# VisualComputingInstitute/RovinaSemanticSegmentation

Hardware: AMD Instinct MI355X
Metric: Mpix/s RF+5-iter DenseCRF @640x480 RGB-D (higher is better)
Workload: dtype f32; 1 GPU; BASELINE configs[2]: batch of 64 synthetic 640x480 RGB-D key frames per GPU (10 % invalid-depth holes: yes; 2 input sets in rotation), 4-tree forest (2^14 leaves/tree, D=366, C=9), RF + 5-iter DenseCRF (d=6, Potts w=10), marginals + labels written to HBM; label_gather=none

## Files before the change

### rovinasemanticsegmentation_amd/csrc/kernels_lattice.hip

```cpp
#include <string.h>

#include <rocprim/rocprim.hpp>

#include "device_math.h"
#include "rvseg_crf.h"

namespace rvseg {

constexpr int ST_EMPTY = -1, ST_LOCKED = -2, ST_FILLED = 0;

struct Key8 {
    union {
        short k[8];
        unsigned w[4];
        unsigned long long q[2];
    };
};

__device__ __forceinline__ unsigned hash_key(const Key8& key) {
    unsigned h = 0x9E3779B9u;
#pragma unroll
    for (int i = 0; i < 4; i++) {
        h ^= key.w[i];
        h *= 0x85EBCA6Bu;
// ... 249 lines not shown
    }
    RV_LAUNCHED("lattice_points_kernel");
}

struct SlotFilled {
    __device__ __forceinline__ int operator()(int st) const { return st == ST_FILLED ? 1 : 0; }
};

__global__ void __launch_bounds__(256)
lattice_compact_kernel(LatticeDev L) {
    const unsigned slot = blockIdx.x * blockDim.x + threadIdx.x;
    if (slot >= L.cap_total) return;
    const bool filled = L.state[slot] == ST_FILLED;
    const int id = L.slot_to_id[slot];
    if (filled && (unsigned)id < (unsigned)L.m_bound) {
        L.vkeys[2 * (size_t)id] = L.tkeys[2 * (size_t)slot];
        L.vkeys[2 * (size_t)id + 1] = L.tkeys[2 * (size_t)slot + 1];
    }
    const unsigned cap_f = L.cap_f_mask + 1;
    if ((slot & L.cap_f_mask) == 0) L.fstart[slot >> L.cap_f_log2] = id;
    if (slot == L.cap_total - 1) {
        const int M = id + (filled ? 1 : 0);
        L.counters[0] = M;
        L.fstart[L.n_frames] = M;
        if (M > L.m_bound) L.counters[1] = 1;
    }
    if ((slot & L.cap_f_mask) == L.cap_f_mask) {
        const int first = L.slot_to_id[slot - L.cap_f_mask];
        const int Mf = id + (filled ? 1 : 0) - first;
        if ((unsigned)Mf > cap_f / 2) L.counters[1] = 1;
    }
}

__global__ void __launch_bounds__(256)
lattice_remap_kernel(LatticeDev L, unsigned* __restrict__ sort_keys, unsigned* __restrict__ sort_vals, long long n_entries) {
    const long long e = (long long)blockIdx.x * blockDim.x + threadIdx.x;
    if (e >= n_entries) return;
    int id = L.slot_to_id[L.offsets[e]];
    id = id < L.m_bound ? id : L.m_bound - 1;
    L.offsets[e] = id;
    sort_keys[e] = (unsigned)id;
    sort_vals[e] = (unsigned)e;
}

__global__ void __launch_bounds__(256)
lattice_neighbours_kernel(LatticeDev L) {
    const long long gid = (long long)blockIdx.x * blockDim.x + threadIdx.x;
    const int M = L.counters[0] < L.m_bound ? L.counters[0] : L.m_bound;
    const int d = L.d;
    if (gid >= (long long)M * (d + 1)) return;
    const int j = (int)(gid / M);
    const int id = (int)(gid - (long long)j * M);
    Key8 key;
    const unsigned long long* src = L.vkeys + 2 * (size_t)id;
    key.q[0] = src[0];
    key.q[1] = src[1];
    Key8 n1 = key, n2 = key;
    for (int k = 0; k < d; k++) { n1.k[k] = (short)(key.k[k] - 1); n2.k[k] = (short)(key.k[k] + 1); }
    if (j < d) { n1.k[j] = (short)(key.k[j] + d); n2.k[j] = (short)(key.k[j] - d); }
    const unsigned fbase = (unsigned)(unsigned short)key.k[7] << L.cap_f_log2;
    const int s1 = hash_lookup(L.state, L.tkeys, fbase, L.cap_f_mask, n1);
    const int s2 = hash_lookup(L.state, L.tkeys, fbase, L.cap_f_mask, n2);
    L.nb1[(size_t)j * L.m_bound + id] = s1 < 0 ? -1 : L.slot_to_id[s1];
    L.nb2[(size_t)j * L.m_bound + id] = s2 < 0 ? -1 : L.slot_to_id[s2];
}

__global__ void __launch_bounds__(256)
lattice_csr_kernel(LatticeDev L, const unsigned* __restrict__ keys_sorted, const unsigned* __restrict__ vals_sorted,
                   long long n_entries) {
    const long long k = (long long)blockIdx.x * blockDim.x + threadIdx.x;
    if (k >= n_entries) return;
    const unsigned e = vals_sorted[k];
    const unsigned key = keys_sorted[k];
    L.csr_pw[k] = make_uint2(e / (unsigned)(L.d + 1), __float_as_uint(L.bary[e]));
    if (k == 0 || keys_sorted[k - 1] != key) L.vstart[key] = (unsigned)k;
    if (k == n_entries - 1 || keys_sorted[k + 1] != key) L.vend[key] = (unsigned)(k + 1);
}

void launch_vertex_order(const LatticeDev& L, SortBuffers& sb, hipStream_t s);

constexpr int CS_PIX_MIN = 256;
constexpr int CS_MCAP = 4096;

template <bool SCATTER>
__global__ void __launch_bounds__(256)
csr_pass_kernel(LatticeDev L, unsigned* __restrict__ bh, int wbpf, int mcap) {
    extern __shared__ unsigned cs_cnt[];
    const int wave = threadIdx.x >> 6, lane = threadIdx.x & 63;
    const long long gwb = (long long)blockIdx.x * 4 + wave;
    const int frame = (int)(gwb / wbpf);
    if (frame >= L.n_frames) return;
    const int wb = (int)(gwb - (long long)frame * wbpf);
    const int f0 = L.fstart[frame] < L.m_bound ? L.fstart[frame] : L.m_bound;
    const int f1 = L.fstart[frame + 1] < L.m_bound ? L.fstart[frame + 1] : L.m_bound;
    const int Mf = f1 - f0 < mcap ? f1 - f0 : mcap;
    const unsigned n_entries_total = (unsigned)((long long)L.n_frames * L.N * (L.d + 1));
    unsigned* my = cs_cnt + (size_t)wave * mcap;
    unsigned* row = bh + (size_t)wbpf * f0 + (size_t)wb * Mf;
    for (int lv = lane; lv < Mf; lv += 64) my[lv] = SCATTER ? row[lv] : 0u;
    if (Mf == 0 && lane == 0) my[0] = 0xFFFFFFFFu;
    __builtin_amdgcn_fence(__ATOMIC_SEQ_CST, "wavefront");
    const int dp1 = L.d + 1;
    const long long p0 = (long long)wb * L.cs_pix;
    const long long p1 = p0 + L.cs_pix < L.N ? p0 + L.cs_pix : L.N;
    const long long ebeg = ((long long)frame * L.N + p0) * dp1, eend = ((long long)frame * L.N + p1) * dp1;
    const unsigned long long lt = lane == 0 ? 0ull : (~0ull >> (64 - lane));
    auto fetch = [&](long long e, int& id, float& wgt) {
        id = 0; wgt = 0.f;
        if (e < eend) {
            if (!SCATTER) { id = L.slot_to_id[L.offsets[e]]; id = id < L.m_bound ? id : L.m_bound - 1; }
            else { id = L.offsets[e]; wgt = L.bary[e]; }
        }
    };
    int id_n; float w_n;
    fetch(ebeg + lane, id_n, w_n);
    for (long long base = ebeg; base < eend; base += 64) {
        const long long e = base + lane;
        const bool valid = e < eend;
        const int id = id_n;
        const float wgt = w_n;
        fetch(e + 64, id_n, w_n);
        if (!SCATTER && valid) L.offsets[e] = id;
        int lv = valid ? id - f0 : -1;
        if (lv >= Mf) lv = Mf - 1;
        if (valid && lv < 0) lv = 0;
        if (!SCATTER) {
            if (valid) atomicAdd(&my[lv], 1u);
            continue;
        }
        bool pending = valid;
        for (;;) {
            const unsigned long long todo = __ballot(pending);
            if (!todo) break;
            const int leader = __ffsll((long long)todo) - 1;
            const int k = __shfl(lv, leader, 64);
            const bool same = pending && lv == k;
            const unsigned long long m = __ballot(same);
            const unsigned c = (unsigned)__popcll(m);
            if (SCATTER) {
                const unsigned b = my[k];
                if (same) {
                    const unsigned pos = b + (unsigned)__popcll(m & lt);
                    if (pos < n_entries_total) {
                        L.csr_pw[pos] = make_uint2((unsigned)(e / dp1), __float_as_uint(wgt));
                    }
                }
                if (lane == leader) my[k] = b + c;
            } else {
                if (lane == leader) my[k] = my[k] + c;
            }
            pending = pending && !same;
        }
        __builtin_amdgcn_fence(__ATOMIC_SEQ_CST, "wavefront");
    }
    if (!SCATTER) {
        for (int lv = lane; lv < Mf; lv += 64) row[lv] = my[lv];
    }
}

__global__ void __launch_bounds__(256)
csr_count_kernel(LatticeDev L, unsigned* __restrict__ bh, int wbpf, int mcap) {
    extern __shared__ unsigned cs_cnt[];
    const int wave = threadIdx.x >> 6, lane = threadIdx.x & 63;
    const long long gwb = (long long)blockIdx.x * 4 + wave;
    const int frame = (int)(gwb / wbpf);
    if (frame >= L.n_frames) return;
    const int wb = (int)(gwb - (long long)frame * wbpf);
    const int f0 = L.fstart[frame] < L.m_bound ? L.fstart[frame] : L.m_bound;
    const int f1 = L.fstart[frame + 1] < L.m_bound ? L.fstart[frame + 1] : L.m_bound;
    const int Mf = f1 - f0 < mcap ? f1 - f0 : mcap;
    unsigned* my = cs_cnt + (size_t)wave * mcap;
    unsigned* row = bh + (size_t)wbpf * f0 + (size_t)wb * Mf;
    for (int lv = lane; lv < Mf; lv += 64) my[lv] = 0u;
    __builtin_amdgcn_fence(__ATOMIC_SEQ_CST, "wavefront");
    const int dp1 = L.d + 1;
    const long long p0 = (long long)wb * L.cs_pix;
    const long long p1 = p0 + L.cs_pix < L.N ? p0 + L.cs_pix : L.N;
    const long long ebeg = ((long long)frame * L.N + p0) * dp1, eend = ((long long)frame * L.N + p1) * dp1;
    auto fetch = [&](long long e, int (&sl)[4]) {
        if (e + 4 <= eend) {
            load_row<4>(L.offsets + e, sl);
        } else {
#pragma unroll
            for (int k = 0; k < 4; k++) sl[k] = e + k < eend ? L.offsets[e + k] : 0;
        }
    };
    int sl_n[4];
    fetch(ebeg + 4 * lane < eend ? ebeg + 4 * lane : ebeg, sl_n);
    for (long long base = ebeg; base < eend; base += 256) {
        const long long e = base + 4 * lane;
        int sl[4], id[4];
#pragma unroll
        for (int k = 0; k < 4; k++) sl[k] = sl_n[k];
        const bool any = e < eend;
        if (any) {
#pragma unroll
            for (int k = 0; k < 4; k++) id[k] = L.slot_to_id[sl[k]];
        }
        const long long en = e + 256;
        fetch(en < eend ? en : ebeg, sl_n);
        if (!any) continue;
#pragma unroll
        for (int k = 0; k < 4; k++) {
            id[k] = id[k] < L.m_bound ? id[k] : L.m_bound - 1;
        }
        if (e + 4 <= eend) {
            store_row<4>(L.offsets + e, id);
        } else {
#pragma unroll
            for (int k = 0; k < 4; k++) if (e + k < eend) L.offsets[e + k] = id[k];
        }
#pragma unroll
        for (int k = 0; k < 4; k++) {
            if (e + k >= eend) continue;
            int lv = id[k] - f0;
            lv = lv < Mf ? lv : Mf - 1;
            lv = lv < 0 ? 0 : lv;
            if (Mf > 0) atomicAdd(&my[lv], 1u);
        }
    }
    __builtin_amdgcn_fence(__ATOMIC_SEQ_CST, "wavefront");
    for (int lv = lane; lv < Mf; lv += 64) row[lv] = my[lv];
}

template <int DP1>
__global__ void __launch_bounds__(256)
csr_scatter_kernel(LatticeDev L, const unsigned* __restrict__ bh, int wbpf, int mcap) {
    extern __shared__ unsigned cs_cnt[];
    const int wave = threadIdx.x >> 6, lane = threadIdx.x & 63;
    const long long gwb = (long long)blockIdx.x * 4 + wave;
    const int frame = (int)(gwb / wbpf);
    if (frame >= L.n_frames) return;
    const int wb = (int)(gwb - (long long)frame * wbpf);
    const int f0 = L.fstart[frame] < L.m_bound ? L.fstart[frame] : L.m_bound;
    const int f1 = L.fstart[frame + 1] < L.m_bound ? L.fstart[frame + 1] : L.m_bound;
    const int Mf = f1 - f0 < mcap ? f1 - f0 : mcap;
    const unsigned n_entries_total = (unsigned)((long long)L.n_frames * L.N * DP1);
    unsigned* my = cs_cnt + (size_t)wave * mcap;
    const unsigned* row = bh + (size_t)wbpf * f0 + (size_t)wb * Mf;
    for (int lv = lane; lv < Mf; lv += 64) my[lv] = row[lv];
    if (Mf == 0 && lane == 0) my[0] = 0xFFFFFFFFu;
    __builtin_amdgcn_fence(__ATOMIC_SEQ_CST, "wavefront");
    const int p0 = wb * L.cs_pix;
    const int p1 = p0 + L.cs_pix < L.N ? p0 + L.cs_pix : L.N;
    const unsigned long long lt = lane == 0 ? 0ull : (~0ull >> (64 - lane));
    for (int pc = p0; pc < p1; pc += 64) {
        const int p = pc + lane;
        const bool valid = p < p1;
        const size_t gp = (size_t)frame * L.N + (valid ? p : p1 - 1);
        int lv[DP1];
        float w[DP1];
        load_row<DP1>(L.offsets + gp * DP1, lv);
        load_row<DP1>(L.bary + gp * DP1, w);
#pragma unroll
        for (int j = 0; j < DP1; j++) {
            lv[j] -= f0;
            lv[j] = lv[j] < Mf ? lv[j] : Mf - 1;
            lv[j] = lv[j] < 0 ? 0 : lv[j];
        }
        unsigned pend = valid ? (1u << DP1) - 1u : 0u;
#pragma unroll
        for (int j = 0; j < DP1; j++) {
            for (;;) {
                const unsigned long long todo = __ballot((pend >> j) & 1u);
                if (!todo) break;
                const int leader = __ffsll((long long)todo) - 1;
                const int k = __builtin_amdgcn_readlane(lv[j], leader);
                unsigned long long all = 0ull;
                float wsel = 0.0f;
                bool hit = false;
#pragma unroll
                for (int jj = j; jj < DP1; jj++) {
                    const bool same = ((pend >> jj) & 1u) && lv[jj] == k;
                    all |= __ballot(same);
                    if (same) { wsel = w[jj]; hit = true; pend &= ~(1u << jj); }
                }
                const unsigned b = my[k];
                if (hit) {
                    const unsigned pos = b + (unsigned)__popcll(all & lt);
                    if (pos < n_entries_total) L.csr_pw[pos] = make_uint2((unsigned)gp, __float_as_uint(wsel));
                }
                if (lane == leader) my[k] = b + (unsigned)__popcll(all);
            }
        }
        __builtin_amdgcn_fence(__ATOMIC_SEQ_CST, "wavefront");
    }
}

constexpr int CS_SEGS = 16;
__device__ __forceinline__ size_t csr_aux_offset(const LatticeDev& L, int wbpf) { return (size_t)wbpf * ((size_t)L.m_bound + 64); }

__global__ void __launch_bounds__(1024)
csr_total_kernel(LatticeDev L, unsigned* __restrict__ bh, int wbpf, int mcap, int n_groups) {
    __shared__ unsigned sseg[CS_SEGS][64];
    const int frame = blockIdx.x / n_groups, grp = blockIdx.x - frame * n_groups;
    const int f0 = L.fstart[frame] < L.m_bound ? L.fstart[frame] : L.m_bound;
    const int f1 = L.fstart[frame + 1] < L.m_bound ? L.fstart[frame + 1] : L.m_bound;
    const int Mf = f1 - f0 < mcap ? f1 - f0 : mcap;
    const int lv0 = grp * 64;
    if (lv0 >= Mf) return;
    const int lvl = threadIdx.x & 63, seg = threadIdx.x >> 6;
    const int sw = (wbpf + CS_SEGS - 1) / CS_SEGS;
    const int w0 = seg * sw, w1 = (w0 + sw < wbpf) ? w0 + sw : wbpf;
    const unsigned* fb = bh + (size_t)wbpf * f0;
    unsigned* vtot = bh + csr_aux_offset(L, wbpf);
    unsigned* segsum = vtot + L.m_bound;
    const int lv = lv0 + lvl;
    const bool ok = lv < Mf;
    unsigned sum = 0;
    if (ok) for (int w = w0; w < w1; w++) sum += fb[(size_t)w * Mf + lv];
    sseg[seg][lvl] = sum;
    if (ok) segsum[(size_t)(f0 + lv) * CS_SEGS + seg] = sum;
    __syncthreads();
    if (seg == 0 && ok) {
        unsigned total = 0;
#pragma unroll
        for (int q = 0; q < CS_SEGS; q++) total += sseg[q][lvl];
        vtot[f0 + lv] = total;
    }
}

__global__ void __launch_bounds__(1024)
csr_scan_kernel(LatticeDev L, unsigned* __restrict__ bh, int wbpf, int mcap, int n_groups) {
    __shared__ unsigned red[16];
    __shared__ unsigned vbase[64];
    const int frame = blockIdx.x / n_groups, grp = blockIdx.x - frame * n_groups;
    const int f0 = L.fstart[frame] < L.m_bound ? L.fstart[frame] : L.m_bound;
    const int f1 = L.fstart[frame + 1] < L.m_bound ? L.fstart[frame + 1] : L.m_bound;
    const int Mf = f1 - f0 < mcap ? f1 - f0 : mcap;
    const int lv0 = grp * 64;
    if (lv0 >= Mf) return;
    const int lvl = threadIdx.x & 63, seg = threadIdx.x >> 6;
    const int sw = (wbpf + CS_SEGS - 1) / CS_SEGS;
    const int w0 = seg * sw, w1 = (w0 + sw < wbpf) ? w0 + sw : wbpf;
    unsigned* fb = bh + (size_t)wbpf * f0;
    const unsigned* vtot = bh + csr_aux_offset(L, wbpf);
    const unsigned* segsum = vtot + L.m_bound;
    const unsigned frame_base = (unsigned)((long long)frame * L.N * (L.d + 1));
    unsigned part = 0;
    for (int v = threadIdx.x; v < lv0; v += 1024) part += vtot[f0 + v];
    for (int off = 32; off > 0; off >>= 1) part += __shfl_xor(part, off, 64);
    if (lvl == 0) red[seg] = part;
    __syncthreads();
    unsigned carry = 0;
#pragma unroll
    for (int q = 0; q < 16; q++) carry += red[q];
    const int lv = lv0 + lvl;
    const bool ok = lv < Mf;
    if (seg == 0) {
        const unsigned total = ok ? vtot[f0 + lv] : 0u;
        unsigned incl = total;
        for (int off = 1; off < 64; off <<= 1) {
            const unsigned t = __shfl_up(incl, off, 64);
            if (lvl >= off) incl += t;
        }
        vbase[lvl] = carry + incl - total;
        if (ok) {
            L.vstart[f0 + lv] = frame_base + carry + incl - total;
            L.vend[f0 + lv] = frame_base + carry + incl;
        }
    }
    __syncthreads();
    if (ok) {
        unsigned run = frame_base + vbase[lvl];
        for (int q = 0; q < seg; q++) run += segsum[(size_t)(f0 + lv) * CS_SEGS + q];
        for (int w = w0; w < w1; w++) {
            const unsigned t = fb[(size_t)w * Mf + lv];
            fb[(size_t)w * Mf + lv] = run;
            run += t;
        }
    }
}

bool csr_fast_path(const LatticeDev& L) { return ((L.cap_f_mask + 1) / 2) <= (unsigned)CS_MCAP; }
size_t csr_fast_bytes(const LatticeDev& L) {
    const size_t wbpf = ((size_t)L.N + L.cs_pix - 1) / L.cs_pix;
    return (wbpf * ((size_t)L.m_bound + 64) + (size_t)L.m_bound * (1 + CS_SEGS)) * sizeof(unsigned);
}

void launch_lattice_finish(const LatticeDev& L, SortBuffers& sb, long long n_entries, hipStream_t s, int phase) {
    const bool fast = csr_fast_path(L) && sb.block_hist;
    if (phase == 2) {
        if (!fast) return;
        const int mcap = (int)((L.cap_f_mask + 1) / 2);
        const int wbpf = (L.N + L.cs_pix - 1) / L.cs_pix;
        const long long waves = (long long)wbpf * L.n_frames;
        const dim3 grid((unsigned)((waves + 3) / 4)), block(256);
        const size_t lds = (size_t)4 * mcap * sizeof(unsigned);
        if (L.d == 6) csr_scatter_kernel<7><<<grid, block, lds, s>>>(L, sb.block_hist, wbpf, mcap);
        else if (L.d == 5) csr_scatter_kernel<6><<<grid, block, lds, s>>>(L, sb.block_hist, wbpf, mcap);
        else if (L.d == 2) csr_scatter_kernel<3><<<grid, block, lds, s>>>(L, sb.block_hist, wbpf, mcap);
        else csr_pass_kernel<true><<<grid, block, lds, s>>>(L, sb.block_hist, wbpf, mcap);
        RV_LAUNCHED("csr_scatter_kernel");
        return;
    }
    const unsigned cap = L.cap_total;
    {
        size_t temp = sb.scan_temp_bytes;
        auto in = rocprim::make_transform_iterator(L.state, SlotFilled());
        (void)rocprim::exclusive_scan(sb.scan_temp, temp, in, L.slot_to_id, 0, (size_t)cap, rocprim::plus<int>(), s);
    }
    lattice_compact_kernel<<<dim3((cap + 255) / 256), dim3(256), 0, s>>>(L);
    const long long nb_threads = (long long)L.m_bound * (L.d + 1);
    lattice_neighbours_kernel<<<dim3((unsigned)((nb_threads + 255) / 256)), dim3(256), 0, s>>>(L);
    RV_LAUNCHED("lattice_compact_kernel / lattice_neighbours_kernel");
    if (fast) {
        const int mcap = (int)((L.cap_f_mask + 1) / 2);
        const int wbpf = (L.N + L.cs_pix - 1) / L.cs_pix;
        const long long waves = (long long)wbpf * L.n_frames;
        const dim3 grid((unsigned)((waves + 3) / 4)), block(256);
        const size_t lds = (size_t)4 * mcap * sizeof(unsigned);
        csr_count_kernel<<<grid, block, lds, s>>>(L, sb.block_hist, wbpf, mcap);
        const int n_groups = (mcap + 63) / 64;
        csr_total_kernel<<<dim3((unsigned)(L.n_frames * n_groups)), dim3(1024), 0, s>>>(L, sb.block_hist, wbpf, mcap, n_groups);
        csr_scan_kernel<<<dim3((unsigned)(L.n_frames * n_groups)), dim3(1024), 0, s>>>(L, sb.block_hist, wbpf, mcap, n_groups);
        RV_LAUNCHED("csr_count_kernel / csr_total_kernel / csr_scan_kernel");
        if (phase == 0) launch_lattice_finish(L, sb, n_entries, s, 2);
    } else {
        lattice_remap_kernel<<<dim3((unsigned)((n_entries + 255) / 256)), dim3(256), 0, s>>>(L, sb.keys_in, sb.vals_in, n_entries);
        size_t temp = sb.temp_bytes;
        (void)rocprim::radix_sort_pairs(sb.temp, temp, sb.keys_in, sb.keys_out, sb.vals_in, sb.vals_out, (size_t)n_entries, 0,
                                        (unsigned)sb.key_bits, s);
        lattice_csr_kernel<<<dim3((unsigned)((n_entries + 255) / 256)), dim3(256), 0, s>>>(L, sb.keys_out, sb.vals_out, n_entries);
        RV_LAUNCHED("lattice_remap_kernel / radix sort / lattice_csr_kernel");
    }
    launch_vertex_order(L, sb, s);
}

__global__ void __launch_bounds__(256)
vertex_len_kernel(LatticeDev L, unsigned* __restrict__ key, unsigned* __restrict__ ids, int len_shift) {
    const int v = blockIdx.x * blockDim.x + threadIdx.x;
    if (v >= L.m_bound) return;
    const int M = L.counters[0] < L.m_bound ? L.counters[0] : L.m_bound;
    unsigned k = 0xFFFFFFFFu;
    if (v < M) {
        atomicMax(&L.counters[3], (int)(L.vend[v] - L.vstart[v]));
        const unsigned len = (L.vend[v] - L.vstart[v]) >> len_shift;
        const unsigned frame = (unsigned)(unsigned short)(L.vkeys[2 * (size_t)v + 1] >> 48);
        k = ((frame < 1023u ? frame : 1022u) << 22) | (0x3FFFFFu - (len < 0x3FFFFFu ? len : 0x3FFFFFu));
    }
    key[v] = k;
    ids[v] = (unsigned)v;
}

void launch_vertex_order(const LatticeDev& L, SortBuffers& sb, hipStream_t s) {
    int len_shift = 0;
    while (((long long)L.N >> len_shift) >= (1 << 22)) len_shift++;
    vertex_len_kernel<<<dim3((unsigned)((L.m_bound + 255) / 256)), dim3(256), 0, s>>>(L, sb.keys_in, sb.vals_in, len_shift);
    size_t temp = sb.temp_bytes;
    (void)rocprim::radix_sort_pairs(sb.temp, temp, sb.keys_in, sb.keys_out, sb.vals_in, L.vorder, (size_t)L.m_bound, 0, 32, s);
    RV_LAUNCHED("vertex_len_kernel / radix sort");
}

size_t scan_temp_bytes(unsigned cap) {
    size_t temp = 0;
    int* nul = nullptr;
    auto in = rocprim::make_transform_iterator(nul, SlotFilled());
    (void)rocprim::exclusive_scan(nullptr, temp, in, nul, 0, (size_t)cap, rocprim::plus<int>(), (hipStream_t)0);
    return temp;
}

size_t sort_temp_bytes(long long n_entries, int key_bits) {
    size_t temp = 0;
    unsigned* nul = nullptr;
    (void)rocprim::radix_sort_pairs(nullptr, temp, nul, nul, nul, nul, (size_t)n_entries, 0, (unsigned)key_bits, (hipStream_t)0);
    return temp;
}

__global__ void __launch_bounds__(256)
csr_norm_kernel(const uint2* __restrict__ csr_pw, const float* __restrict__ norm, float* __restrict__ csr_nrm, long long n_entries,
                const int* __restrict__ counters) {
    if (counters[1]) return;
    const long long k = (long long)blockIdx.x * blockDim.x + threadIdx.x;
    if (k < n_entries) csr_nrm[k] = norm[csr_pw[k].x];
}

void launch_csr_norm(const LatticeDev& L, long long n_entries, hipStream_t s) {
    csr_norm_kernel<<<dim3((unsigned)((n_entries + 255) / 256)), dim3(256), 0, s>>>(L.csr_pw, L.norm, L.csr_nrm, n_entries, L.counters);
    RV_LAUNCHED("csr_norm_kernel");
}
int csr_pix_min() { return CS_PIX_MIN; }

}
```

### rovinasemanticsegmentation_amd/csrc/rvseg_crf.h

```cpp
#pragma once
#include <hip/hip_runtime.h>

#include <cstdint>

#include "rvseg_internal.h"

namespace rvseg {

struct LatticeDev {
    int d;
    int N;
    int Npad;
    int n_frames;
    unsigned cap_f_mask;
    unsigned cap_f_log2;
    unsigned cap_total;
    int m_bound;
    float scale[8];
    int* state;
    unsigned long long* tkeys;
    int* slot_to_id;
    int* counters;
    int* fstart;
    unsigned long long* vkeys;
    int* offsets;
    float* bary;
    int *nb1, *nb2;
    uint2* csr_pw;
    float* csr_nrm;
    unsigned *vstart, *vend;
    unsigned* vorder;
    int n_groups;
    int group_vertices;
    int ordered_sum_scan;
    int cs_pix;
    unsigned heavy_from;
    unsigned scan_ranks;
    const unsigned* bh;
    int wbpf;
    float* norm;
};

constexpr int RES_MAXB = 16;
constexpr int RES_MAX_OWNV = 640;
constexpr int RES_MAX_VERTS = 4096;
constexpr int RES_MAX_BANDS = 512;
struct SplatResidentDev {
    unsigned* tdesc;
    unsigned short* tvl;
    unsigned* tinfo;
    unsigned* blk_tile0;
    unsigned short* blk_verts;
    unsigned* blk_nown;
    unsigned* jb_tile;
    unsigned* prog;
    int* flags;
    unsigned long long* trace;
    int B, band_wb, n_bands, window;
    int chunk_log2;
    unsigned cap_tiles;
};

struct FeatureSource {
    int mode;
    const float* feat;
    const float4* cloud;
    const uint8_t* rgb;
    float xyz_kernel, rgb_kernel;
};

struct ValueView {
    float* base;
    size_t frame_stride;
    size_t layer_off;
    __host__ __device__ __forceinline__ size_t index(unsigned p, int c, int C, int N) const {
        const unsigned frame = p / (unsigned)N;
        const unsigned i = p - frame * (unsigned)N;
        return (size_t)frame * frame_stride + layer_off + (size_t)i * C + c;
    }
    __device__ __forceinline__ float at(unsigned p, int c, int C, int N) const { return base[index(p, c, C, N)]; }
    __device__ __forceinline__ float& ref(unsigned p, int c, int C, int N) const { return base[index(p, c, C, N)]; }
};

struct SortBuffers {
    unsigned *keys_in, *keys_out, *vals_in, *vals_out;
    void* temp;
    size_t temp_bytes;
    int key_bits;
    void* scan_temp;
    size_t scan_temp_bytes;
    unsigned* block_hist;
};

void launch_fill_int(int* p, int v, long long n, hipStream_t s);
void launch_lattice_points(const LatticeDev& L, const FeatureSource& fs, hipStream_t s);
void launch_lattice_finish(const LatticeDev& L, SortBuffers& sb, long long n_entries, hipStream_t s, int phase = 0);
size_t sort_temp_bytes(long long n_entries, int key_bits);
size_t scan_temp_bytes(unsigned cap);
bool csr_fast_path(const LatticeDev& L);
size_t csr_fast_bytes(const LatticeDev& L);
int csr_pix_min();
void launch_csr_norm(const LatticeDev& L, long long n_entries, hipStream_t s);
void launch_splat(const LatticeDev& L, const ValueView& src, int C, int mode, float* values, hipStream_t s, bool own_q = false,
                  const SplatResidentDev* resident = nullptr, int slot = 0);
unsigned splat_walk_items(const LatticeDev& L, int per_item);
void launch_resident_plan(const LatticeDev& L, const SplatResidentDev& r, hipStream_t s);
int resident_block_capacity(int chunk);
int resident_cu_count();
bool launch_splat_resident(const LatticeDev& L, const SplatResidentDev& R, int C, const float* src, float* values, int slot,
                           hipStream_t s);
float* launch_blur(const LatticeDev& L, int C, bool seq, bool reverse, float* a, float* b, hipStream_t s, bool small_blocks = false);
void launch_slice(const LatticeDev& L, int C, bool seq, int out_mode, const float* values, float neg_w, float* out,
                  long long n_points, hipStream_t s);
struct MfLabels {
    int8_t* labels;
    int mode, unknown, n_layers, layer;
};
struct MfTerm {
    float neg_w;
    const float* compat;
    bool matrix, post;
};
bool mf_fused_supported(int C);
bool launch_mf_update(const LatticeDev& L, int C, const float* values, const MfTerm& term, const ValueView& unary, bool negate,
                      const ValueView& Q, bool scale_out, const MfLabels& lab, hipStream_t s);
void launch_neg_unary(const ValueView& unary, bool negate, int C, int N, float* tmp, long long n_points, hipStream_t s);
bool launch_softmax_unary(const ValueView& unary, bool negate, int C, int N, const ValueView& q, long long n_points,
                          const float* scale, hipStream_t s);
void launch_softmax(const float* tmp, int C, int N, const ValueView& q, long long n_points, hipStream_t s);
void launch_term_update(const LatticeDev& L, int C, bool seq, const float* values, bool post, bool matrix, const float* compat,
                        float* tmp, long long n_points, hipStream_t s);
struct KernelParams { float p[49]; };
void launch_kernel_params(const float* f, int N, int d, int kind, const KernelParams& kp, float* out, hipStream_t s);
void launch_logistic_unary(const float* Lm, const float* f, int N, int C, int K, float* U, hipStream_t s);

}
```

### rovinasemanticsegmentation_amd/csrc/rvseg_crf.hip

```cpp
#include <cmath>
#include <cstdio>
#include <cstdlib>
#include <cstring>

#include "rvseg_crf.h"
#include "rvseg_pipeline.h"

namespace rvseg {

struct LatticeBufs {
    DevBuf state, tkeys, slot_to_id, counters, vkeys, offsets, bary, nb1, nb2, csr_pw, csr_nrm, vstart, vend, norm;
    DevBuf keys_in, keys_out, vals_in, vals_out, sort_temp, scan_temp, fstart, vorder, block_hist;
    DevBuf r_desc, r_vl, r_info, r_small, r_verts, r_jb, r_trace;
    SplatResidentDev resident{};
    bool resident_on = false;
    LatticeDev dev{};
    SortBuffers sb{};
    long long n_entries = 0, n_points = 0;
    bool built = false;
    bool cleared = false;
    bool has_csr_nrm = false;
};

struct CrfState {
// ... 46 lines not shown
    int want = ctx->params.lattice_capacity_log2;
    if (safe || want < 0) return safe_log2;
    if (want == 0) want = 12;
    if (ctx->impl) want += ctx->impl->cap_boost;
    return want < safe_log2 ? want : safe_log2;
}

static bool capacity_is_worst_case(const rvseg_ctx* ctx, int N, int d) {
    const int Npad = (N + 3) / 4 * 4;
    return capacity_log2_per_frame(ctx, Npad, d, false) == capacity_log2_per_frame(ctx, Npad, d, true);
}

static bool resident_pays(int n_frames, int N, int vertices_per_frame_seen) {
    const long long vpf = vertices_per_frame_seen > 0 ? vertices_per_frame_seen : 360;
    return n_frames >= 2 && (long long)n_frames * N >= 6900000ll + 4900ll * vpf;
}

static rvseg_status lattice_prepare(rvseg_ctx* ctx, LatticeBufs& b, int d, int N, int n_frames, bool safe, int vertices_per_frame_seen = 0) {
    if (d < 1 || d > 7) { ctx->err = "feature dimension must be in [1,7]"; return RVSEG_ERR_INVALID_ARG; }
    if (n_frames > 1022) { ctx->err = "at most 1022 frames per chunk (lower max_batch)"; return RVSEG_ERR_INVALID_ARG; }
    const int Npad = (N + 3) / 4 * 4;
    const int cap_f_log2 = capacity_log2_per_frame(ctx, Npad, d, safe);
    const unsigned long long cap = (unsigned long long)n_frames << cap_f_log2;
    if (cap >= (1ull << 31)) { ctx->err = "lattice hash capacity too large (lower max_batch or lattice_capacity_log2)"; return RVSEG_ERR_CAPACITY; }
    const unsigned long long worst = (unsigned long long)Npad * n_frames * (d + 1);
    const unsigned long long m_bound = std::min<unsigned long long>(cap / 2 + 2, worst);
    const long long P = (long long)N * n_frames;
    const long long E = P * (d + 1);
    if (E >= (1ll << 32) || m_bound >= (1ull << 31)) { ctx->err = "too many lattice entries for 32-bit indices"; return RVSEG_ERR_CAPACITY; }
    rvseg_status st;
#define RV_RES(buf, bytes) if ((st = dev_reserve(ctx, buf, (size_t)(bytes))) != RVSEG_OK) return st
    RV_RES(b.state, cap * 4);
    RV_RES(b.tkeys, cap * 16);
    RV_RES(b.slot_to_id, cap * 4);
    RV_RES(b.fstart, ((size_t)n_frames + 1) * 4);
    RV_RES(b.vkeys, m_bound * 16);
    RV_RES(b.offsets, E * 4);
    RV_RES(b.bary, E * 4);
    RV_RES(b.nb1, m_bound * (d + 1) * 4);
    RV_RES(b.nb2, m_bound * (d + 1) * 4);
    RV_RES(b.csr_pw, E * 8);
    RV_RES(b.vstart, (2 * m_bound + 4) * 4);
    RV_RES(b.vorder, m_bound * 4);
    RV_RES(b.norm, P * 4);
    const unsigned long long SE = std::max<unsigned long long>((unsigned long long)E, m_bound);
    RV_RES(b.keys_in, SE * 4);
    RV_RES(b.keys_out, SE * 4);
    RV_RES(b.vals_in, SE * 4);
    RV_RES(b.vals_out, SE * 4);
    const int key_bits = std::max(1, ceil_log2(m_bound));
    const size_t temp = std::max(sort_temp_bytes(E, key_bits), sort_temp_bytes((long long)m_bound, 32));
    RV_RES(b.sort_temp, temp);
    const size_t stemp = scan_temp_bytes((unsigned)cap);
    RV_RES(b.scan_temp, stemp);
#undef RV_RES
    LatticeDev& L = b.dev;
    L.d = d; L.N = N; L.Npad = Npad; L.n_frames = n_frames;
    L.cap_f_log2 = (unsigned)cap_f_log2;
    L.cap_f_mask = (1u << cap_f_log2) - 1u;
    L.cap_total = (unsigned)cap;
    L.m_bound = (int)m_bound;
    const float inv_std_dev = (float)(std::sqrt(2.0 / 3.0) * (d + 1));
    for (int i = 0; i < 8; i++) L.scale[i] = i < d ? (float)(1.0 / std::sqrt((double)((i + 2) * (i + 1))) * inv_std_dev) : 0.f;
    L.state = b.state.as<int>(); L.tkeys = b.tkeys.as<unsigned long long>(); L.slot_to_id = b.slot_to_id.as<int>();
    L.fstart = b.fstart.as<int>(); L.vkeys = b.vkeys.as<unsigned long long>();
    L.offsets = b.offsets.as<int>(); L.bary = b.bary.as<float>();
    L.nb1 = b.nb1.as<int>(); L.nb2 = b.nb2.as<int>();
    L.csr_pw = b.csr_pw.as<uint2>(); L.csr_nrm = nullptr;
    b.has_csr_nrm = false;
    L.vstart = b.vstart.as<unsigned>(); L.vend = L.vstart + m_bound; L.counters = reinterpret_cast<int*>(L.vend + m_bound);
    L.vorder = b.vorder.as<unsigned>(); L.norm = b.norm.as<float>();
    L.n_groups = n_frames >= 8 ? 8 : 1;
    b.sb.keys_in = b.keys_in.as<unsigned>(); b.sb.keys_out = b.keys_out.as<unsigned>();
    b.sb.vals_in = b.vals_in.as<unsigned>(); b.sb.vals_out = b.vals_out.as<unsigned>();
    b.sb.temp = b.sort_temp.p; b.sb.temp_bytes = temp; b.sb.key_bits = key_bits;
    b.sb.scan_temp = b.scan_temp.p; b.sb.scan_temp_bytes = stemp;
    b.sb.block_hist = nullptr;
    L.bh = nullptr; L.wbpf = 0;
    L.group_vertices = ctx->sched.group_vertices;
    L.ordered_sum_scan = ctx->sched.serial_chains ? 0 : 1;
    L.heavy_from = 0;
    L.scan_ranks = 0;
    L.cs_pix = ctx->sched.csr_block > 0 ? ctx->sched.csr_block : (n_frames <= 8 ? 256 : 1024);
    if (csr_fast_path(L)) {
        if ((st = dev_reserve(ctx, b.block_hist, csr_fast_bytes(L))) != RVSEG_OK) return st;
        b.sb.block_hist = b.block_hist.as<unsigned>();
        L.bh = b.sb.block_hist;
        L.wbpf = (N + L.cs_pix - 1) / L.cs_pix;
    }
    b.n_entries = E; b.n_points = P;
    b.built = false;
    b.cleared = false;
    b.resident_on = false;
    {
        const rvseg_schedule& sc = ctx->sched;
        const bool wanted = sc.splat == 2 || (sc.splat == 0 && resident_pays(n_frames, N, vertices_per_frame_seen));
        const int chunk = sc.resident_chunk == 64 ? 64 : 128;
        const int capacity = resident_block_capacity(chunk);
        int B = sc.resident_blocks > 0 ? sc.resident_blocks : (n_frames > 0 ? resident_cu_count() / n_frames : 0);
        if (sc.resident_blocks <= 0) B = B < 2 ? 2 : (B > 12 ? 12 : B);
        B = B > RES_MAXB ? RES_MAXB : B;
        if (wanted && L.bh && d == 6 && B >= 2 && (long long)n_frames * B <= capacity &&
            7ll * N < (1ll << 24) && (long long)L.wbpf * L.cs_pix <= 8192ll * RES_MAX_BANDS && L.cs_pix <= 4096) {
            SplatResidentDev& R = b.resident;
            R.B = B;
            R.band_wb = sc.resident_band < 1 ? 1 : (sc.resident_band > 32 ? 32 : sc.resident_band);
            R.band_wb = std::max(1, R.band_wb * 256 / L.cs_pix);
            R.n_bands = (L.wbpf + R.band_wb - 1) / R.band_wb;
            while (R.n_bands > RES_MAX_BANDS) { R.band_wb *= 2; R.n_bands = (L.wbpf + R.band_wb - 1) / R.band_wb; }
            R.window = sc.resident_window;
            R.chunk_log2 = chunk == 128 ? 7 : 6;
            R.cap_tiles = (unsigned)(N / 8 + 1024);
            if (sc.resident_cap_tiles > 0 && (unsigned)sc.resident_cap_tiles < R.cap_tiles) R.cap_tiles = (unsigned)sc.resident_cap_tiles;
            const size_t small = (16 + (size_t)n_frames * (RES_MAXB + 1) + (size_t)n_frames * RES_MAXB + 2 * (size_t)n_frames * RES_MAXB) * 4;
            if ((st = dev_reserve(ctx, b.r_desc, (size_t)n_frames * 7 * R.cap_tiles * 4)) != RVSEG_OK) return st;
            if ((st = dev_reserve(ctx, b.r_vl, (size_t)n_frames * 7 * R.cap_tiles * 2)) != RVSEG_OK) return st;
            if ((st = dev_reserve(ctx, b.r_info, (size_t)n_frames * R.cap_tiles * 4)) != RVSEG_OK) return st;
            if ((st = dev_reserve(ctx, b.r_small, small)) != RVSEG_OK) return st;
            if ((st = dev_reserve(ctx, b.r_verts, (size_t)n_frames * RES_MAXB * RES_MAX_OWNV * 2)) != RVSEG_OK) return st;
            if ((st = dev_reserve(ctx, b.r_jb, (size_t)n_frames * RES_MAXB * (R.n_bands + 1) * 4)) != RVSEG_OK) return st;
            R.tdesc = b.r_desc.as<unsigned>(); R.tvl = b.r_vl.as<unsigned short>(); R.tinfo = b.r_info.as<unsigned>();
            unsigned* sm = b.r_small.as<unsigned>();
            R.flags = reinterpret_cast<int*>(sm); sm += 16;
            R.blk_tile0 = sm; sm += (size_t)n_frames * (RES_MAXB + 1);
            R.blk_nown = sm; sm += (size_t)n_frames * RES_MAXB;
            R.prog = sm;
            R.blk_verts = b.r_verts.as<unsigned short>();
            R.jb_tile = b.r_jb.as<unsigned>();
            R.trace = nullptr;
            if (sc.trace) {
                if ((st = dev_reserve(ctx, b.r_trace, (size_t)n_frames * RES_MAXB * 64)) != RVSEG_OK) return st;
                R.trace = b.r_trace.as<unsigned long long>();
            }
            b.resident_on = true;
        }
    }
    return RVSEG_OK;
}

static rvseg_status values_reserve(rvseg_ctx* ctx, CrfState* cs, long long m_bound, int C, int slot = 0) {
    rvseg_status st;
    if ((st = dev_reserve(ctx, cs->scratch[slot].val_a, (size_t)m_bound * C * 4)) != RVSEG_OK) return st;
    if ((st = dev_reserve(ctx, cs->scratch[slot].val_b, (size_t)m_bound * C * 4)) != RVSEG_OK) return st;
    return RVSEG_OK;
}

static rvseg_status second_stream(rvseg_ctx* ctx, CrfState* cs) {
    if (cs->layer_stream) return RVSEG_OK;
    int prio_lo = 0, prio_hi = 0;
    (void)hipDeviceGetStreamPriorityRange(&prio_lo, &prio_hi);
    Stream stream;
    Event fork, join;
    RV_HIP(ctx, stream_create(stream, hipStreamNonBlocking, prio_hi));
    RV_HIP(ctx, event_create(fork, hipEventDisableTiming));
    RV_HIP(ctx, event_create(join, hipEventDisableTiming));
    cs->layer_stream = std::move(stream);
    cs->layer_fork = std::move(fork);
    cs->layer_join = std::move(join);
    return RVSEG_OK;
}

static rvseg_status lattice_clear(rvseg_ctx* ctx, LatticeBufs& b, hipStream_t s) {
    const LatticeDev& L = b.dev;
    RV_HIP(ctx, hipMemsetAsync(L.state, 0xFF, (size_t)L.cap_total * 4, s));
    RV_HIP(ctx, hipMemsetAsync(L.vstart, 0, (2 * (size_t)L.m_bound + 4) * 4, s));
    b.cleared = true;
// ... 797 lines not shown
```

Before: 1758 Mpix/s.

## Size CSR LDS histogram to observed vertex count and tile vertex range

The CSR count and scatter kernels now size their per-wave LDS histogram from the observed vertices per frame instead of the worst-case capacity. Frames with more vertices than fit are handled by looping over vertex windows, or by falling back to global atomics in the count kernel. The change also forces 8 waves per EU on the scatter kernels. Smaller LDS footprints should raise occupancy, at the cost of rescanning entries once per window and slower global atomics when a frame overflows.

Result: no change. 1755 Mpix/s (-0.2%).

```diff
diff --git a/rovinasemanticsegmentation_amd/csrc/kernels_lattice.hip b/rovinasemanticsegmentation_amd/csrc/kernels_lattice.hip
--- a/rovinasemanticsegmentation_amd/csrc/kernels_lattice.hip
+++ b/rovinasemanticsegmentation_amd/csrc/kernels_lattice.hip
@@ -355,9 +355,18 @@
 constexpr int CS_PIX_MIN = 256;
 constexpr int CS_MCAP = 4096;
 
-template <bool SCATTER>
-__global__ void __launch_bounds__(256)
-csr_pass_kernel(LatticeDev L, unsigned* __restrict__ bh, int wbpf, int mcap) {
+constexpr int CS_LDS_FLOOR = 512;
+
+int csr_lds_rows(const LatticeDev& L, int vertices_per_frame_seen) {
+    const int mcap = (int)((L.cap_f_mask + 1) / 2);
+    if (vertices_per_frame_seen <= 0) return mcap;
+    int m = CS_LDS_FLOOR;
+    while (m < mcap && m < 2 * (long long)vertices_per_frame_seen) m <<= 1;
+    return m < mcap ? m : mcap;
+}
+
+__global__ void __launch_bounds__(256) __attribute__((amdgpu_waves_per_eu(8, 8)))
+csr_pass_kernel(LatticeDev L, const unsigned* __restrict__ bh, int wbpf, int mcap) {
     extern __shared__ unsigned cs_cnt[];
     const int wave = threadIdx.x >> 6, lane = threadIdx.x & 63;
     const long long gwb = (long long)blockIdx.x * 4 + wave;
@@ -367,12 +376,10 @@
     const int f0 = L.fstart[frame] < L.m_bound ? L.fstart[frame] : L.m_bound;
     const int f1 = L.fstart[frame + 1] < L.m_bound ? L.fstart[frame + 1] : L.m_bound;
     const int Mf = f1 - f0 < mcap ? f1 - f0 : mcap;
+    const int lds_m = L.lds_m;
     const unsigned n_entries_total = (unsigned)((long long)L.n_frames * L.N * (L.d + 1));
-    unsigned* my = cs_cnt + (size_t)wave * mcap;
-    unsigned* row = bh + (size_t)wbpf * f0 + (size_t)wb * Mf;
-    for (int lv = lane; lv < Mf; lv += 64) my[lv] = SCATTER ? row[lv] : 0u;
-    if (Mf == 0 && lane == 0) my[0] = 0xFFFFFFFFu;
-    __builtin_amdgcn_fence(__ATOMIC_SEQ_CST, "wavefront");
+    unsigned* my = cs_cnt + (size_t)wave * lds_m;
+    const unsigned* row = bh + (size_t)wbpf * f0 + (size_t)wb * Mf;
     const int dp1 = L.d + 1;
     const long long p0 = (long long)wb * L.cs_pix;
     const long long p1 = p0 + L.cs_pix < L.N ? p0 + L.cs_pix : L.N;
@@ -380,37 +387,34 @@
     const unsigned long long lt = lane == 0 ? 0ull : (~0ull >> (64 - lane));
     auto fetch = [&](long long e, int& id, float& wgt) {
         id = 0; wgt = 0.f;
-        if (e < eend) {
-            if (!SCATTER) { id = L.slot_to_id[L.offsets[e]]; id = id < L.m_bound ? id : L.m_bound - 1; }
-            else { id = L.offsets[e]; wgt = L.bary[e]; }
-        }
+        if (e < eend) { id = L.offsets[e]; wgt = L.bary[e]; }
     };
-    int id_n; float w_n;
-    fetch(ebeg + lane, id_n, w_n);
-    for (long long base = ebeg; base < eend; base += 64) {
-        const long long e = base + lane;
-        const bool valid = e < eend;
-        const int id = id_n;
-        const float wgt = w_n;
-        fetch(e + 64, id_n, w_n);
-        if (!SCATTER && valid) L.offsets[e] = id;
-        int lv = valid ? id - f0 : -1;
-        if (lv >= Mf) lv = Mf - 1;
-        if (valid && lv < 0) lv = 0;
-        if (!SCATTER) {
-            if (valid) atomicAdd(&my[lv], 1u);
-            continue;
-        }
-        bool pending = valid;
-        for (;;) {
-            const unsigned long long todo = __ballot(pending);
-            if (!todo) break;
-            const int leader = __ffsll((long long)todo) - 1;
-            const int k = __shfl(lv, leader, 64);
-            const bool same = pending && lv == k;
-            const unsigned long long m = __ballot(same);
-            const unsigned c = (unsigned)__popcll(m);
-            if (SCATTER) {
+    for (int v0 = 0; v0 == 0 || v0 < Mf; v0 += lds_m) {
+        const int vn = Mf - v0 < lds_m ? Mf - v0 : lds_m;
+        for (int lv = lane; lv < vn; lv += 64) my[lv] = row[v0 + lv];
+        if (Mf == 0 && lane == 0) my[0] = 0xFFFFFFFFu;
+        __builtin_amdgcn_fence(__ATOMIC_SEQ_CST, "wavefront");
+        int id_n; float w_n;
+        fetch(ebeg + lane, id_n, w_n);
+        for (long long base = ebeg; base < eend; base += 64) {
+            const long long e = base + lane;
+            const bool valid = e < eend;
+            const int id = id_n;
+            const float wgt = w_n;
+            fetch(e + 64, id_n, w_n);
+            int lv = valid ? id - f0 : -1;
+            if (lv >= Mf) lv = Mf - 1;
+            if (valid && lv < 0) lv = 0;
+            lv -= v0;
+            bool pending = valid && (unsigned)lv < (unsigned)lds_m;
+            for (;;) {
+                const unsigned long long todo = __ballot(pending);
+                if (!todo) break;
+                const int leader = __ffsll((long long)todo) - 1;
+                const int k = __shfl(lv, leader, 64);
+                const bool same = pending && lv == k;
+                const unsigned long long m = __ballot(same);
+                const unsigned c = (unsigned)__popcll(m);
                 const unsigned b = my[k];
                 if (same) {
                     const unsigned pos = b + (unsigned)__popcll(m & lt);
@@ -419,15 +423,10 @@
                     }
                 }
                 if (lane == leader) my[k] = b + c;
-            } else {
-                if (lane == leader) my[k] = my[k] + c;
+                pending = pending && !same;
             }
-            pending = pending && !same;
-        }
-        __builtin_amdgcn_fence(__ATOMIC_SEQ_CST, "wavefront");
-    }
-    if (!SCATTER) {
-        for (int lv = lane; lv < Mf; lv += 64) row[lv] = my[lv];
+            __builtin_amdgcn_fence(__ATOMIC_SEQ_CST, "wavefront");
+        }
     }
 }
 
@@ -442,10 +441,16 @@
     const int f0 = L.fstart[frame] < L.m_bound ? L.fstart[frame] : L.m_bound;
     const int f1 = L.fstart[frame + 1] < L.m_bound ? L.fstart[frame + 1] : L.m_bound;
     const int Mf = f1 - f0 < mcap ? f1 - f0 : mcap;
-    unsigned* my = cs_cnt + (size_t)wave * mcap;
+    const bool in_lds = Mf <= L.lds_m;
+    unsigned* my = cs_cnt + (size_t)wave * L.lds_m;
     unsigned* row = bh + (size_t)wbpf * f0 + (size_t)wb * Mf;
-    for (int lv = lane; lv < Mf; lv += 64) my[lv] = 0u;
-    __builtin_amdgcn_fence(__ATOMIC_SEQ_CST, "wavefront");
+    if (in_lds) {
+        for (int lv = lane; lv < Mf; lv += 64) my[lv] = 0u;
+        __builtin_amdgcn_fence(__ATOMIC_SEQ_CST, "wavefront");
+    } else {
+        for (int lv = lane; lv < Mf; lv += 64) row[lv] = 0u;
+        __builtin_amdgcn_fence(__ATOMIC_RELEASE, "agent");
+    }
     const int dp1 = L.d + 1;
     const long long p0 = (long long)wb * L.cs_pix;
     const long long p1 = p0 + L.cs_pix < L.N ? p0 + L.cs_pix : L.N;
@@ -489,15 +494,18 @@
             int lv = id[k] - f0;
             lv = lv < Mf ? lv : Mf - 1;
             lv = lv < 0 ? 0 : lv;
-            if (Mf > 0) atomicAdd(&my[lv], 1u);
-        }
-    }
+            if (Mf <= 0) continue;
+            if (in_lds) atomicAdd(&my[lv], 1u);
+            else (void)__hip_atomic_fetch_add(&row[lv], 1u, __ATOMIC_RELAXED, __HIP_MEMORY_SCOPE_AGENT);
+        }
+    }
+    if (!in_lds) return;
     __builtin_amdgcn_fence(__ATOMIC_SEQ_CST, "wavefront");
     for (int lv = lane; lv < Mf; lv += 64) row[lv] = my[lv];
 }
 
 template <int DP1>
-__global__ void __launch_bounds__(256)
+__global__ void __launch_bounds__(256) __attribute__((amdgpu_waves_per_eu(8, 8)))
 csr_scatter_kernel(LatticeDev L, const unsigned* __restrict__ bh, int wbpf, int mcap) {
     extern __shared__ unsigned cs_cnt[];
     const int wave = threadIdx.x >> 6, lane = threadIdx.x & 63;
@@ -509,14 +517,17 @@
     const int f1 = L.fstart[frame + 1] < L.m_bound ? L.fstart[frame + 1] : L.m_bound;
     const int Mf = f1 - f0 < mcap ? f1 - f0 : mcap;
     const unsigned n_entries_total = (unsigned)((long long)L.n_frames * L.N * DP1);
-    unsigned* my = cs_cnt + (size_t)wave * mcap;
+    const int lds_m = L.lds_m;
+    unsigned* my = cs_cnt + (size_t)wave * lds_m;
     const unsigned* row = bh + (size_t)wbpf * f0 + (size_t)wb * Mf;
-    for (int lv = lane; lv < Mf; lv += 64) my[lv] = row[lv];
-    if (Mf == 0 && lane == 0) my[0] = 0xFFFFFFFFu;
-    __builtin_amdgcn_fence(__ATOMIC_SEQ_CST, "wavefront");
     const int p0 = wb * L.cs_pix;
     const int p1 = p0 + L.cs_pix < L.N ? p0 + L.cs_pix : L.N;
     const unsigned long long lt = lane == 0 ? 0ull : (~0ull >> (64 - lane));
+  for (int v0 = 0; v0 == 0 || v0 < Mf; v0 += lds_m) {
+    const int vn = Mf - v0 < lds_m ? Mf - v0 : lds_m;
+    for (int t = lane; t < vn; t += 64) my[t] = row[v0 + t];
+    if (Mf == 0 && lane == 0) my[0] = 0xFFFFFFFFu;
+    __builtin_amdgcn_fence(__ATOMIC_SEQ_CST, "wavefront");
     for (int pc = p0; pc < p1; pc += 64) {
         const int p = pc + lane;
         const bool valid = p < p1;
@@ -530,8 +541,11 @@
             lv[j] -= f0;
             lv[j] = lv[j] < Mf ? lv[j] : Mf - 1;
             lv[j] = lv[j] < 0 ? 0 : lv[j];
-        }
-        unsigned pend = valid ? (1u << DP1) - 1u : 0u;
+            lv[j] -= v0;
+        }
+        unsigned pend = 0u;
+#pragma unroll
+        for (int j = 0; j < DP1; j++) pend |= (valid && (unsigned)lv[j] < (unsigned)lds_m) ? 1u << j : 0u;
 #pragma unroll
         for (int j = 0; j < DP1; j++) {
             for (;;) {
@@ -558,6 +572,7 @@
         }
         __builtin_amdgcn_fence(__ATOMIC_SEQ_CST, "wavefront");
     }
+  }
 }
 
 constexpr int CS_SEGS = 16;
@@ -570,26 +585,27 @@
     const int f0 = L.fstart[frame] < L.m_bound ? L.fstart[frame] : L.m_bound;
     const int f1 = L.fstart[frame + 1] < L.m_bound ? L.fstart[frame + 1] : L.m_bound;
     const int Mf = f1 - f0 < mcap ? f1 - f0 : mcap;
-    const int lv0 = grp * 64;
-    if (lv0 >= Mf) return;
     const int lvl = threadIdx.x & 63, seg = threadIdx.x >> 6;
     const int sw = (wbpf + CS_SEGS - 1) / CS_SEGS;
     const int w0 = seg * sw, w1 = (w0 + sw < wbpf) ? w0 + sw : wbpf;
     const unsigned* fb = bh + (size_t)wbpf * f0;
     unsigned* vtot = bh + csr_aux_offset(L, wbpf);
     unsigned* segsum = vtot + L.m_bound;
-    const int lv = lv0 + lvl;
-    const bool ok = lv < Mf;
-    unsigned sum = 0;
-    if (ok) for (int w = w0; w < w1; w++) sum += fb[(size_t)w * Mf + lv];
-    sseg[seg][lvl] = sum;
-    if (ok) segsum[(size_t)(f0 + lv) * CS_SEGS + seg] = sum;
-    __syncthreads();
-    if (seg == 0 && ok) {
-        unsigned total = 0;
-#pragma unroll
-        for (int q = 0; q < CS_SEGS; q++) total += sseg[q][lvl];
-        vtot[f0 + lv] = total;
+    for (int lv0 = grp * 64; lv0 < Mf; lv0 += n_groups * 64) {
+        const int lv = lv0 + lvl;
+        const bool ok = lv < Mf;
+        unsigned sum = 0;
+        if (ok) for (int w = w0; w < w1; w++) sum += fb[(size_t)w * Mf + lv];
+        sseg[seg][lvl] = sum;
+        if (ok) segsum[(size_t)(f0 + lv) * CS_SEGS + seg] = sum;
+        __syncthreads();
+        if (seg == 0 && ok) {
+            unsigned total = 0;
+#pragma unroll
+            for (int q = 0; q < CS_SEGS; q++) total += sseg[q][lvl];
+            vtot[f0 + lv] = total;
+        }
+        __syncthreads();
     }
 }
 
@@ -601,8 +617,6 @@
     const int f0 = L.fstart[frame] < L.m_bound ? L.fstart[frame] : L.m_bound;
     const int f1 = L.fstart[frame + 1] < L.m_bound ? L.fstart[frame + 1] : L.m_bound;
     const int Mf = f1 - f0 < mcap ? f1 - f0 : mcap;
-    const int lv0 = grp * 64;
-    if (lv0 >= Mf) return;
     const int lvl = threadIdx.x & 63, seg = threadIdx.x >> 6;
     const int sw = (wbpf + CS_SEGS - 1) / CS_SEGS;
     const int w0 = seg * sw, w1 = (w0 + sw < wbpf) ? w0 + sw : wbpf;
@@ -610,6 +624,7 @@
     const unsigned* vtot = bh + csr_aux_offset(L, wbpf);
     const unsigned* segsum = vtot + L.m_bound;
     const unsigned frame_base = (unsigned)((long long)frame * L.N * (L.d + 1));
+  for (int lv0 = grp * 64; lv0 < Mf; lv0 += n_groups * 64) {
     unsigned part = 0;
     for (int v = threadIdx.x; v < lv0; v += 1024) part += vtot[f0 + v];
     for (int off = 32; off > 0; off >>= 1) part += __shfl_xor(part, off, 64);
@@ -643,6 +658,8 @@
             run += t;
         }
     }
+    __syncthreads();
+  }
 }
 
 bool csr_fast_path(const LatticeDev& L) { return ((L.cap_f_mask + 1) / 2) <= (unsigned)CS_MCAP; }
@@ -659,11 +676,11 @@
         const int wbpf = (L.N + L.cs_pix - 1) / L.cs_pix;
         const long long waves = (long long)wbpf * L.n_frames;
         const dim3 grid((unsigned)((waves + 3) / 4)), block(256);
-        const size_t lds = (size_t)4 * mcap * sizeof(unsigned);
+        const size_t lds = (size_t)4 * L.lds_m * sizeof(unsigned);
         if (L.d == 6) csr_scatter_kernel<7><<<grid, block, lds, s>>>(L, sb.block_hist, wbpf, mcap);
         else if (L.d == 5) csr_scatter_kernel<6><<<grid, block, lds, s>>>(L, sb.block_hist, wbpf, mcap);
         else if (L.d == 2) csr_scatter_kernel<3><<<grid, block, lds, s>>>(L, sb.block_hist, wbpf, mcap);
-        else csr_pass_kernel<true><<<grid, block, lds, s>>>(L, sb.block_hist, wbpf, mcap);
+        else csr_pass_kernel<<<grid, block, lds, s>>>(L, sb.block_hist, wbpf, mcap);
         RV_LAUNCHED("csr_scatter_kernel");
         return;
     }
@@ -682,9 +699,9 @@
         const int wbpf = (L.N + L.cs_pix - 1) / L.cs_pix;
         const long long waves = (long long)wbpf * L.n_frames;
         const dim3 grid((unsigned)((waves + 3) / 4)), block(256);
-        const size_t lds = (size_t)4 * mcap * sizeof(unsigned);
+        const size_t lds = (size_t)4 * L.lds_m * sizeof(unsigned);
         csr_count_kernel<<<grid, block, lds, s>>>(L, sb.block_hist, wbpf, mcap);
-        const int n_groups = (mcap + 63) / 64;
+        const int n_groups = (L.lds_m + 63) / 64;
         csr_total_kernel<<<dim3((unsigned)(L.n_frames * n_groups)), dim3(1024), 0, s>>>(L, sb.block_hist, wbpf, mcap, n_groups);
         csr_scan_kernel<<<dim3((unsigned)(L.n_frames * n_groups)), dim3(1024), 0, s>>>(L, sb.block_hist, wbpf, mcap, n_groups);
         RV_LAUNCHED("csr_count_kernel / csr_total_kernel / csr_scan_kernel");
diff --git a/rovinasemanticsegmentation_amd/csrc/rvseg_crf.h b/rovinasemanticsegmentation_amd/csrc/rvseg_crf.h
--- a/rovinasemanticsegmentation_amd/csrc/rvseg_crf.h
+++ b/rovinasemanticsegmentation_amd/csrc/rvseg_crf.h
@@ -34,6 +34,7 @@
     int group_vertices;
     int ordered_sum_scan;
     int cs_pix;
+    int lds_m;
     unsigned heavy_from;
     unsigned scan_ranks;
     const unsigned* bh;
@@ -98,6 +99,7 @@
 size_t sort_temp_bytes(long long n_entries, int key_bits);
 size_t scan_temp_bytes(unsigned cap);
 bool csr_fast_path(const LatticeDev& L);
+int csr_lds_rows(const LatticeDev& L, int vertices_per_frame_seen);
 size_t csr_fast_bytes(const LatticeDev& L);
 int csr_pix_min();
 void launch_csr_norm(const LatticeDev& L, long long n_entries, hipStream_t s);
diff --git a/rovinasemanticsegmentation_amd/csrc/rvseg_crf.hip b/rovinasemanticsegmentation_amd/csrc/rvseg_crf.hip
--- a/rovinasemanticsegmentation_amd/csrc/rvseg_crf.hip
+++ b/rovinasemanticsegmentation_amd/csrc/rvseg_crf.hip
@@ -152,6 +152,7 @@
     L.heavy_from = 0;
     L.scan_ranks = 0;
     L.cs_pix = ctx->sched.csr_block > 0 ? ctx->sched.csr_block : (n_frames <= 8 ? 256 : 1024);
+    L.lds_m = csr_lds_rows(L, vertices_per_frame_seen);
     if (csr_fast_path(L)) {
         if ((st = dev_reserve(ctx, b.block_hist, csr_fast_bytes(L))) != RVSEG_OK) return st;
         b.sb.block_hist = b.block_hist.as<unsigned>();
```
